# awikner/SPEEDY-ML-1

Hardware: AMD Instinct MI355X
Metric: hybrid timesteps/sec, T30L8 + 1152x6k-node reservoirs; 1/2/4/8-GPU scaling (higher is better)
Workload: dtype f64

## Files before the change

include/speedy_ml.h:

```cpp
#ifndef SPEEDY_ML_H
#define SPEEDY_ML_H

#include <stddef.h>
#include <stdint.h>

#ifdef __cplusplus
extern "C" {
#endif

#define SML_OK 0
#define SML_ERR_ARG (-1)
#define SML_ERR_HIP (-2)
#define SML_ERR_NOMEM (-3)
#define SML_ERR_STATE (-4)
#define SML_ERR_IO (-5)
#define SML_ERR_FORMAT (-6)

#define SML_F32 1
#define SML_F64 2

#define SML_MX 31
#define SML_NX 32
#define SML_MX2 62
#define SML_IX 96
// ... 59 lines not shown
#define SML_RES_PATH_PER_REGION 2
#define SML_RES_PATH_UNGROUPED_FINISH 4
#define SML_RES_PATH_STEPWISE_DRIVE 8
#define SML_RES_PATH_RADIUS_GLOBAL 16
int sml_res_set_reference_paths(sml_reservoirs *c, int flags);
#define SML_RADIUS_OK 0
#define SML_RADIUS_MAXITER 1
#define SML_RADIUS_ZERO 2
#define SML_RADIUS_INVALID 3
int sml_res_spectral_radius(sml_reservoirs *c, double tol, int max_iter, double *lo, double *hi, int *iters,
                            int *info, void *stream);
int sml_gen_region(int n, int k, int ninp, uint64_t seed, int region, double sigma, int *rows, int *cols,
                   float *vals, int *win_col, float *win_val);
int sml_res_set_update_cus(sml_reservoirs *c, int cus);
int sml_res_update_balanced(sml_reservoirs *c, int *balanced);
int sml_res_ell_layout(sml_reservoirs *c, int i, int *a_width, int *a_overflow, int *win_q, int *win_ell);
int sml_res_set_begin_mode(sml_reservoirs *c, int mode);
int sml_res_begin_fused(const sml_reservoirs *c, int *fused);
int sml_res_synchronize(sml_reservoirs *c, const double *d_inputs, int length, int64_t stride, void *stream);
int sml_res_start_prediction(sml_reservoirs *c, const double *d_inputs, int length, int64_t stride,
                             double *d_feedback, void *stream);
int sml_res_train_drive(sml_reservoirs *c, const double *d_inputs, int m, int64_t stride, const double *d_model,
                        int64_t model_stride, double *d_states, double *d_targets, void *stream);
int sml_res_step_host(sml_reservoirs *c, const double *feedback, const double *local_model, double *outvec);
int sml_res_footprint(const sml_reservoirs *c, int64_t *weight_bytes, int64_t *algorithmic_bytes_per_step);
int sml_res_enable_timing(sml_reservoirs *c, int capacity);
int sml_res_kernel_times(sml_reservoirs *c, float *update_ms, float *readout_ms, int max_steps, int *count);
#define SML_RES_MAX_MEMBERS 32
int sml_res_set_members(sml_reservoirs *c, int members);
int sml_res_members(const sml_reservoirs *c, int *members);
// ... 222 lines not shown
```

speedy-ml-1_amd/csrc/sml_res_rows.hpp:

```cpp
#pragma once
#include <hip/hip_runtime.h>

#include <cstdint>

#include "sml_reservoir_layout.hpp"

#ifndef SML_UPD_NT
#define SML_UPD_NT 1
#endif

namespace {
using namespace sml;

__device__ inline int xcd_remap(int b, int nb) {
    const int q8 = nb / 8, rem = nb % 8, xcd = b % 8, idx = b / 8;
    return xcd * q8 + min(xcd, rem) + idx;
}

struct Ell {
    const uint16_t *a_col;
    const void *a_val;
    const uint16_t *w_col;
    const void *w_val;
    const uint64_t *a_om;
// ... 65 lines not shown
        const int np = (rg.a_w + 1) >> 1, n = rg.n;
#pragma unroll
        for (int p = 0; p < kEllA / 2; ++p)
            if (p < np) load_pair<WT, kNT>(q, p, cb + (size_t)p * n + i, vb + 2 * ((size_t)p * n + i));
        if (rg.a_ov) {
            q.om = row_load<kNT>(ell.a_om + rg.a_om + (i >> 6));
            q.ob = row_load<kNT>(ell.a_ob + rg.a_om + (i >> 6));
        }
    }
    if (live && rg.w_w > 0) {
        q.wc = rg.w_q > 0 ? win_col_implicit(rg, i) : (uint32_t)row_load<kNT>(ell.w_col + rg.w_ell + i);
        q.wv = row_load<kNT>((const WT *)ell.w_val + rg.w_ell + i);
    }
}

template <typename WT, int NP, bool OVF>
__device__ inline void load_row_fixed(RowRegs<WT> &q, const RegionDev &rg, const Ell &ell, int i) {
    const uint32_t *cb = reinterpret_cast<const uint32_t *>(ell.a_col + rg.a_ell);
    const WT *vb = (const WT *)ell.a_val + rg.a_ell;
    const uint32_t *zc = reinterpret_cast<const uint32_t *>(ell.zero);
    const WT *zv = reinterpret_cast<const WT *>(ell.zero);
    const int np = (rg.a_w + 1) >> 1, n = rg.n;
    if (OVF) {
        q.om = 0;
        q.ob = 0;
        if (rg.a_ov) {
            q.om = stream_load(ell.a_om + rg.a_om + (i >> 6));
            q.ob = stream_load(ell.a_ob + rg.a_om + (i >> 6));
        }
    }
#pragma unroll
    for (int p = 0; p < NP; ++p) {
        const bool in = p < np;
        load_pair(q, p, in ? cb + (size_t)p * n + i : zc, in ? vb + 2 * ((size_t)p * n + i) : zv);
    }
    if (rg.w_q > 0)
        q.wc = win_col_implicit(rg, i);
    else
        q.wc = stream_load(ell.w_col + rg.w_ell + i);
    q.wv = stream_load((const WT *)ell.w_val + rg.w_ell + i);
}

template <typename WT, bool kFixed>
__device__ inline void resolve_ovf(RowRegs<WT> &q, const RegionDev &rg, const Ell &ell, int i) {
    const int b = i & 63;
    const uint64_t below = b ? q.om << (64 - b) : 0ull;
    q.oh = rg.a_ov && ((q.om >> b) & 1ull);
    const int64_t e = rg.a_oe + q.ob + __popcll(below);
    if (q.oh) {
        q.oc = kFixed ? stream_load(ell.a_oc + e) : ell.a_oc[e];
        q.ov = kFixed ? stream_load((const WT *)ell.a_ov + e) : ((const WT *)ell.a_ov)[e];
    }
}

__device__ __attribute__((always_inline)) inline double res_tanh(double x) {
    double a = fabs(x);
    a = a > 20.0 ? 20.0 : a;
    const double em = expm1(2.0 * a);
    return copysign(em / (em + 2.0), x);
}

template <typename WT>
__device__ inline int ell_col(const RowRegs<WT> &q, int s) {
    return (int)((q.c[s >> 1] >> (16 * (s & 1))) & 0xffffu);
}

template <typename WT>
__device__ __attribute__((always_inline)) inline double ell_row_value(const RowRegs<WT> &q, const RegionDev &rg,
                                                                      const double *xs, const double *fs, int i,
                                                                      double leak) {
    double y = 0.0;
#pragma unroll
    for (int s = 0; s < kEllA; ++s)
        if (s < rg.a_w) y = y + (double)q.v[s] * xs[ell_col(q, s)];
    if (q.oh) y = y + (double)q.ov * xs[q.oc];
    double t = 0.0;
    t = t + (double)q.wv * fs[q.wc];
    const double xn = res_tanh(y + t);
    return (1.0 - leak) * xs[i] + leak * xn;
}

template <typename WT>
struct CsrRows {
    const int32_t *rp;
    const uint16_t *ac;
    const WT *av;
    const int32_t *wp;
    const uint16_t *wc;
    const WT *wv;
};

template <typename WT>
__device__ __attribute__((always_inline)) inline double row_value(RowRegs<WT> &cur, const RegionDev &rg,
                                                                  const Ell &ell, const CsrRows<WT> &csr,
                                                                  const double *xs, const double *fs, int i,
                                                                  double leak) {
    double y = 0.0;
    if (rg.a_w > 0) {
        cur.oh = false;
        if (rg.a_ov) resolve_ovf<WT, false>(cur, rg, ell, i);
#pragma unroll
        for (int s = 0; s < kEllA; ++s)
            if (s < rg.a_w) y = y + (double)cur.v[s] * xs[ell_col(cur, s)];
        if (cur.oh) y = y + (double)cur.ov * xs[cur.oc];
    } else {
        for (int e = csr.rp[i], e1 = csr.rp[i + 1]; e < e1; ++e) y = y + (double)csr.av[e] * xs[csr.ac[e]];
    }
    double t = 0.0;
    if (rg.w_w > 0) {
        t = t + (double)cur.wv * fs[cur.wc];
    } else {
        for (int e = csr.wp[i], e1 = csr.wp[i + 1]; e < e1; ++e) t = t + (double)csr.wv[e] * fs[csr.wc[e]];
    }
    const double xn = res_tanh(y + t);
    return (1.0 - leak) * xs[i] + leak * xn;
// ... 43 lines not shown
```

speedy-ml-1_amd/csrc/sml_res_update.hpp:

```cpp
#pragma once
#include <hip/hip_runtime.h>

#include <cstdint>

#include "sml_res_rows.hpp"
#include "sml_reservoir_layout.hpp"
#include "sml_timeline.hpp"

namespace {
using namespace sml;

template <typename WT, bool kLds, int kMinW = 4>
__global__ __launch_bounds__(kUpdThreads, kMinW) void k_res_update(
    const RegionDev *__restrict__ R, const int32_t *__restrict__ a_rp, const uint16_t *__restrict__ a_col,
    const WT *__restrict__ a_val, const int32_t *__restrict__ w_rp, const uint16_t *__restrict__ w_col,
    const WT *__restrict__ w_val, Ell ell, const double *__restrict__ x_old, double *__restrict__ x_new,
    const double *__restrict__ feedback, double leak, int parts, int lds_x, int nlog) {
    SML_TL_SCOPE(sml::tl::kUpdate);
    extern __shared__ __attribute__((aligned(16))) double smem[];
    const int off = xcd_remap(blockIdx.x, gridDim.x);
    for (int base = 0; base < nlog; base += gridDim.x) {
        const int lb = base + off;
        if (lb < nlog)
            update_block<WT, kLds>(lb, smem, R, a_rp, a_col, a_val, w_rp, w_col, w_val, ell, x_old, x_new,
                                   feedback, leak, parts, lds_x);
        if (base + (int)gridDim.x < nlog) __syncthreads();
    }
}

struct PassDesc {
    int r, base, end, seg;
    bool live;
};

struct StageRegs {
    double x[kStageX];
    double f;
};

template <typename WT, int NP, bool OVF, int kDepth = 2>
__global__ __launch_bounds__(kUpdThreads, 4) void k_res_update_bal(
    const RegionDev *__restrict__ R, const int32_t *__restrict__ row0, const int32_t *__restrict__ blk_r0, int nlocal,
    int64_t total, Ell ell, const double *__restrict__ x_old, double *__restrict__ x_new,
    const double *__restrict__ feedback, double leak, int lds_x, int lds_buf) {
    SML_TL_SCOPE(sml::tl::kUpdate);
    extern __shared__ __attribute__((aligned(16))) double smem[];
    const int G = gridDim.x;
    const int b = xcd_remap(blockIdx.x, G);
    const int g0 = (int)(total * b / G), g1 = (int)(total * (b + 1) / G);
    if (g0 >= g1) return;
    const int tid = threadIdx.x;
    auto seg_at = [&](int r, int seg) -> PassDesc {
        const int a = row0[r], e = row0[r + 1];
        return PassDesc{r, max(g0, a) - a, min(g1, e) - a, seg, true};
    };
    auto succ = [&](const PassDesc &p) -> PassDesc {
        if (!p.live) return p;
        if (p.base + kUpdThreads < p.end) return PassDesc{p.r, p.base + kUpdThreads, p.end, p.seg, true};
        const int r = p.r + 1;
        if (r >= nlocal || row0[r] >= g1) return PassDesc{r, 0, 0, p.seg + 1, false};
        return seg_at(r, p.seg + 1);
    };
    auto load = [&](RowRegs<WT> &q, const PassDesc &p) {
        if (!p.live) return;
        const RegionDev rg = R[p.r];
        const int i = p.base + tid;
        load_row_fixed<WT, NP, OVF>(q, rg, ell, i < p.end ? i : 0);
    };
    auto resolve = [&](RowRegs<WT> &q, const PassDesc &p) {
        q.oh = false;
        if (!OVF || !p.live) return;
        const RegionDev rg = R[p.r];
        if (!rg.a_ov) return;
        const int i = p.base + tid;
        resolve_ovf<WT, true>(q, rg, ell, i < p.end ? i : 0);
    };
    auto stage_load = [&](StageRegs &sr, int r) {
        const RegionDev rg = R[r];
        const double *xo = x_old + rg.x;
#pragma unroll
        for (int q = 0; q < kStageX; ++q) {
            const int j = tid + q * kUpdThreads;
            if (j < rg.n) sr.x[q] = xo[j];
        }
        if (tid < rg.ninp) sr.f = feedback[rg.fb + tid];
    };
    auto stage_store = [&](const StageRegs &sr, int r, double *buf) {
        const RegionDev rg = R[r];
#pragma unroll
        for (int q = 0; q < kStageX; ++q) {
            const int j = tid + q * kUpdThreads;
            if (j < rg.n) buf[j] = sr.x[q];
        }
        if (tid < rg.ninp) buf[lds_x + tid] = sr.f;
    };
    static_assert(kDepth == 2 || kDepth == 3, "update pipeline depth");
    PassDesc P0 = seg_at(blk_r0[b], 0);
    RowRegs<WT> L0, L1, L2, L3;
    load(L0, P0);
    resolve(L0, P0);
    PassDesc P1 = succ(P0);
    load(L1, P1);
    PassDesc P2 = succ(P1), P3 = P2;
    if constexpr (kDepth == 3) {
        load(L2, P2);
        P3 = succ(P2);
    }
    {
        StageRegs sr;
        stage_load(sr, P0.r);
        stage_store(sr, P0.r, smem);
    }
    __syncthreads();
    while (P0.live) {
        resolve(L1, P1);
        if constexpr (kDepth == 3)
            load(L3, P3);
        else
            load(L2, P2);
        const bool newseg = P1.live && P1.seg != P0.seg;
        StageRegs sr;
        if (newseg) stage_load(sr, P1.r);
        {
            const RegionDev rg = R[P0.r];
            const double *xs = smem + (size_t)(P0.seg & 1) * lds_buf, *fs = xs + lds_x;
            const int i = P0.base + tid;
            if (i < P0.end) x_new[rg.x + i] = ell_row_value(L0, rg, xs, fs, i, leak);
        }
        if (newseg) {
            stage_store(sr, P1.r, smem + (size_t)(P1.seg & 1) * lds_buf);
            __syncthreads();
        }
        P0 = P1;
        L0 = L1;
        P1 = P2;
        L1 = L2;
        if constexpr (kDepth == 3) {
            P2 = P3;
            L2 = L3;
            P3 = succ(P3);
        } else {
            P2 = succ(P2);
        }
    }
}

}
```

speedy-ml-1_amd/csrc/sml_reservoir.hip:

```cpp
#include <hip/hip_ext.h>
#include <hip/hip_runtime.h>

#include <algorithm>
#include <cmath>
#include <cstdlib>
#include <cstring>
#include <memory>
#include <new>
#include <type_traits>
#include <vector>

#include "sml_devmem.hpp"
#include "sml_internal.hpp"
#include "sml_reservoir_layout.hpp"
#include "sml_timeline.hpp"

SML_TL_DEFINE(reservoir)

#include "sml_res_rows.hpp"
#include "sml_res_update.hpp"
#include "sml_res_drive.hpp"
#include "sml_res_radius.hpp"
#include "sml_res_tiling.hpp"
#include "sml_res_readout.hpp"
// ... 51 lines not shown
    bool stepwise_drive = false;
    bool radius_global = false;
    double *d_rad_xy = nullptr, *d_rad_part = nullptr;
    RadiusOut *d_rad_out = nullptr;
    StepShape shape;
    int members = 1;
    MemberShape mshape;
    MemberFinish mfin;
    int fin_tile_want = 0;
    int32_t *d_tgt_idx = nullptr;
    const uint64_t *fin_wflag = nullptr;
    uint64_t fin_wval = 0;
    unsigned *fin_wlate = nullptr;
    long long fin_wtimeout = 400000000ll;
    int upd_cus = 0, ncu = 0;
    std::vector<int32_t> blk_off;
    std::vector<std::vector<int32_t>> blk_host;
    int blk_cap = 0;
    size_t max_lds = 0;
    int32_t *d_row0 = nullptr, *d_blk_r0 = nullptr;
    std::vector<int32_t> row0_h;
    int8_t *d_outl = nullptr;
    int32_t *d_asm_dst = nullptr;
    int32_t *d_fb_src = nullptr;
    uint8_t *d_fb_l = nullptr;
    uint16_t *d_fb_reg = nullptr;
    int tot_tisr = 0;
    int32_t *d_tisr_fb = nullptr, *d_tisr_grid = nullptr;
    uint16_t *d_tisr_reg = nullptr;
    int32_t *d_lm_src = nullptr;
    uint8_t *d_lm_l = nullptr;
    double *d_io = nullptr;
    size_t d_io_n = 0;
    StepEvents timers;
    std::vector<double> meanstd_h;
// ... 261 lines not shown
        for (int l = 0; l < kMeanStd; ++l) c->meanstd_h[(size_t)i * 2 * kMeanStd + kMeanStd + l] = 1.0;
    int rc;
    if ((rc = upload(c->d_rd, c->rd)) || (rc = upload(c->d_meanstd, c->meanstd_h)) || (rc = build_tables(c)) ||
        (rc = upload(c->d_row0, c->row0_h)))
        return rc;
    *out = owner.release();
    return SML_OK;
}

Ell make_ell(const sml_reservoirs *c) {
    return Ell{c->d_a_ell_col, c->d_a_ell_val, c->d_w_ell_col, c->d_w_ell_val, c->d_a_om,
               c->d_a_ob,      c->d_a_oc,      c->d_a_ov,      c->d_zero};
}


int launch_update_bal(sml_reservoirs *c, const double *xo, double *xn, const double *d_feedback, hipStream_t st) {
    const StepShape &s = c->shape;
    const int64_t total = c->row0_h[c->nlocal];
    int G = c->upd_cus > 0 ? c->upd_cus : std::max(c->ncu, 1);
    G = (int)std::max<int64_t>(1, std::min<int64_t>(G, total));
    if (G > c->blk_cap) {
        const int cap = std::max(G, std::max(c->ncu, c->upd_cus));
        if (c->d_blk_r0) {
            SML_HIP(hipDeviceSynchronize());
            c->mem.release(&c->d_blk_r0);
            c->blk_cap = 0;
        }
        if (int rc = pool(c, &c->d_blk_r0, (int64_t)cap * (cap + 1) / 2)) return rc;
        c->blk_off.assign(cap + 1, -1);
        c->blk_cap = cap;
    }
    if (c->blk_off[G] < 0) {
        c->blk_off[G] = G * (G - 1) / 2;
        c->blk_host.push_back(block_first_regions(c->row0_h, G));
        SML_HIP(hipMemcpyAsync(c->d_blk_r0 + c->blk_off[G], c->blk_host.back().data(), (size_t)G * 4,
                               hipMemcpyHostToDevice, st));
    }
    const int32_t *blk_r0 = c->d_blk_r0 + c->blk_off[G];
    const Ell ell = make_ell(c);
    int np = 2;
    bool ovf = false;
    for (int i = 0; i < c->nlocal; ++i) {
        np = std::max(np, (c->rd[i].a_w + 1) / 2);
        ovf = ovf || c->rd[i].a_ov;
    }
    auto go = [&](auto kern) {
        hipLaunchKernelGGL(kern, dim3(G), dim3(kUpdThreads), s.lds_bal, st, c->d_rd, c->d_row0, blk_r0, c->nlocal,
                           total, ell, xo, xn, d_feedback, c->leakage, s.lds_x, s.lds_buf);
    };
    with_wt(c, [&](auto tag) {
        using WT = decltype(tag);
        if (np == 2) ovf ? go(k_res_update_bal<WT, 2, true, 2>) : go(k_res_update_bal<WT, 2, false, 2>);
        else if (np == 3) ovf ? go(k_res_update_bal<WT, 3, true, 2>) : go(k_res_update_bal<WT, 3, false, 2>);
        else ovf ? go(k_res_update_bal<WT, 4, true, 2>) : go(k_res_update_bal<WT, 4, false, 2>);
    });
    SML_HIP(hipGetLastError());
    return SML_OK;
}

int launch_update(sml_reservoirs *c, const double *xo, double *xn, const double *d_feedback, hipStream_t st) {
    const StepShape &s = c->shape;
    if (s.balanced) return launch_update_bal(c, xo, xn, d_feedback, st);
    const int nlog = s.parts * c->nlocal;
    const Ell ell = make_ell(c);
    with_wt(c, [&](auto tag) {
        using WT = decltype(tag);
        auto go = [&](auto kern, size_t shared) {
            hipLaunchKernelGGL(kern, dim3(nlog), dim3(kUpdThreads), shared, st, c->d_rd, c->d_a_rp, c->d_a_col,
                               (const WT *)c->d_a_val, c->d_w_rp, c->d_w_col, (const WT *)c->d_w_val, ell, xo, xn,
// ... 348 lines not shown
    return SML_OK;
}

extern "C" int sml_res_set_update_cus(sml_reservoirs *c, int cus) {
    SML_REQUIRE(c && cus >= 0, "bad argument");
    c->upd_cus = cus;
    return SML_OK;
}

extern "C" int sml_res_update_balanced(sml_reservoirs *c, int *balanced) {
    SML_REQUIRE(c && balanced, "null argument");
    *balanced = c->shape.balanced ? 1 : 0;
    return SML_OK;
}

extern "C" int sml_res_ell_layout(sml_reservoirs *c, int i, int *a_width, int *a_overflow, int *win_q,
                                  int *win_ell) {
    if (int rc = check_region(c, i)) return rc;
    SML_REQUIRE(a_width && a_overflow && win_q && win_ell, "null argument");
    const RegionDev &r = c->rd[i];
    *a_width = r.a_w;
    *a_overflow = r.a_ov;
    *win_q = r.w_q;
    *win_ell = r.w_w;
    return SML_OK;
}

extern "C" int sml_res_set_reference_paths(sml_reservoirs *c, int flags) {
    SML_REQUIRE(c && (flags & ~31) == 0, "bad argument");
    const bool csr = flags & SML_RES_PATH_CSR;
// ... 679 lines not shown
```

speedy-ml-1_amd/csrc/sml_reservoir_layout.cpp:

```cpp
#include "sml_reservoir_layout.hpp"

#include <algorithm>

namespace sml {

PoolPlan plan_pools(const PoolPlanIn &in) {
    PoolPlan p;
    p.rd.resize(in.nlocal);
    p.ld.resize(in.nlocal);
    for (int i = 0; i < in.nlocal; ++i) {
        const int n = in.n[i];
        p.ld[i] = (in.ncs + n + kLdAlign - 1) / kLdAlign * kLdAlign;
        RegionDev &r = p.rd[i];
        r.n = n;
        r.ninp = in.ninp[i];
        r.ld = p.ld[i];
        r.a_rp = p.tot_a_rp;
        p.tot_a_rp += n + 1;
        r.a_nz = p.tot_a_nz;
        p.tot_a_nz += in.k[i];
        r.w_rp = p.tot_w_rp;
        p.tot_w_rp += n + 1;
        r.w_nz = p.tot_w_nz;
        p.tot_w_nz += n;
// ... 317 lines not shown
        std::copy(t.begin(), t.begin() + cnt, tidx.begin() + (size_t)i * nout);
    }
    return SML_OK;
}

std::vector<int32_t> block_first_regions(const std::vector<int32_t> &row0, int G) {
    const int64_t total = row0.back();
    std::vector<int32_t> r0(G);
    for (int b = 0; b < G; ++b) {
        const int64_t g0 = total * b / G;
        r0[b] = (int32_t)(std::upper_bound(row0.begin(), row0.end(), (int32_t)g0) - row0.begin() - 1);
    }
    return r0;
}

void footprint(int nlocal, const int *nn, const int *kk, const int *ni, int ncs, int nout, int64_t wb,
               int64_t *weight_bytes, int64_t *algo_bytes) {
    int64_t w = 0, a = 0;
    for (int i = 0; i < nlocal; ++i) {
        const int64_t n = nn[i], k = kk[i], ninp = ni[i];
        const int64_t wout = wb * nout * (ncs + n);
        const int64_t amat = 4 * (n + 1) + (2 + wb) * k;
        const int64_t winm = 4 * (n + 1) + (2 + wb) * n;
        w += wout + amat + winm;
        a += wout + amat + winm + 8 * n + 8 * n + 8 * ninp + 8 * ncs + 8 * nout;
    }
    if (weight_bytes) *weight_bytes = w;
    if (algo_bytes) *algo_bytes = a;
}

// ... 2 lines not shown
```

speedy-ml-1_amd/csrc/sml_reservoir_layout.hpp:

```cpp
#pragma once

#include <cstdint>
#include <vector>

#include "sml_internal.hpp"

namespace sml {

constexpr int kLdAlign = 32;
constexpr int kRows = 8;
constexpr int kMeanStd = 36;
constexpr int kTisrStride = 16;
constexpr int kSrcKeep = -1;

constexpr int kEllA = 8;
constexpr int kEllW = 1;

struct RegionDev {
    int n, ninp, ld;
    int a_w, w_w;
    int a_ov;
    int w_q;
    uint32_t w_magic;
    int64_t a_rp, a_nz, w_rp, w_nz, wout, x, xaug, fb;
// ... 149 lines not shown
    std::vector<uint16_t> fb_reg;
    std::vector<int32_t> lm_src;
    std::vector<uint8_t> lm_l;
    std::vector<int32_t> tisr_fb, tisr_grid;
    std::vector<uint16_t> tisr_reg;
    std::vector<int8_t> outl;
    std::vector<int32_t> tgt_idx;
};

int build_region_tables(const TablesIn &in, RegionTables *out);

int out_std_index(int o, const RegionGeom &g);

std::vector<int32_t> block_first_regions(const std::vector<int32_t> &row0, int G);

void footprint(int nlocal, const int *n, const int *k, const int *ninp, int ncs, int nout, int64_t wb,
               int64_t *weight_bytes, int64_t *algo_bytes);

}
```

speedy-ml-1_amd/speedy_ml_amd/_lib.py:

```python
from __future__ import annotations

import ctypes
import os
import subprocess

PKG_ROOT = os.path.dirname(os.path.dirname(os.path.abspath(__file__)))
LIB_PATH = os.environ.get("SML_LIB") or os.path.join(PKG_ROOT, "lib", "libspeedyml.so")
CSRC = os.path.join(PKG_ROOT, "csrc")

SML_OK = 0
SML_F32 = 1
SML_F64 = 2

EXPORTED = (
    "sml_last_error", "sml_abi_version",
    "sml_spectral_create", "sml_spectral_destroy", "sml_spectral_tables",
    "sml_grid_batched", "sml_spec_batched", "sml_gridy_batched", "sml_gridx_batched",
    "sml_specx_batched", "sml_specy_batched", "sml_vdspec_batched", "sml_uvspec_batched",
    "sml_grid_host", "sml_spec_host",
    "sml_res_create", "sml_res_destroy", "sml_res_ninp", "sml_res_feedback_offsets",
    "sml_res_load_region_f32", "sml_res_load_region_f64", "sml_res_set_state", "sml_res_get_state",
    "sml_res_step", "sml_res_step_begin", "sml_res_step_finish", "sml_res_step_finish_grid", "sml_res_step_finish_assemble", "sml_res_step_host", "sml_res_synchronize",
    "sml_res_footprint", "sml_res_enable_timing", "sml_res_kernel_times", "sml_res_set_read_waves",
    "sml_res_set_begin_mode", "sml_res_begin_fused",
# ... 12 lines not shown
    "sml_dyn_run_model", "sml_dyn_last_safe", "sml_dyn_set_check_cus", "sml_res_info",
    "sml_comm_unique_id", "sml_comm_create", "sml_comm_create_file", "sml_comm_destroy", "sml_comm_rank",
    "sml_comm_allgather",
    "sml_hybrid_create", "sml_hybrid_destroy", "sml_hybrid_set_buffers", "sml_hybrid_set_tisr",
    "sml_hybrid_streams", "sml_hybrid_cus", "sml_hybrid_start", "sml_hybrid_predict", "sml_hybrid_advance", "sml_hybrid_step",
    "sml_hybrid_run_speedy", "sml_hybrid_sync",
    "sml_device_alloc", "sml_device_free", "sml_copy_to_device", "sml_copy_to_host", "sml_region_geometry",
    "sml_processor_decomposition", "sml_hybrid_set_tisr_table", "sml_tisr_date_index", "sml_res_tile_tisr_field",
    "sml_res_create_generic", "sml_res_step_slab", "sml_res_start_prediction",
    "sml_comm_create_local", "sml_exchange_plan", "sml_hybrid_advance_slabs", "sml_hybrid_set_hop_mode",
    "sml_hybrid_hop_mode", "sml_calendar_delta_hour", "sml_hybrid_set_feb29", "sml_hybrid_get_feb29",
    "sml_res_mean_std", "sml_res_set_outvec_ld", "sml_hybrid_set_slab", "sml_hybrid_start_slab",
    "sml_hybrid_exchange_width", "sml_hybrid_slab_buffers", "sml_dyn_set_hybrid_sst", "sml_dyn_set_sea_ice",
    "sml_hybrid_set_pipelined", "sml_res_step_cancel", "sml_res_step_begun", "sml_hybrid_set_force_exchange",
    "sml_hybrid_exchanges", "sml_hybrid_set_chain", "sml_hybrid_chain", "sml_hybrid_exchange_stream",
    "sml_res_set_update_cus", "sml_res_update_balanced", "sml_probe_mfma_f64_clock", "sml_res_ell_layout",
    "sml_dyn_get_sea_ice", "sml_dyn_get_physics", "sml_dyn_get_forcing", "sml_dyn_set_surface",
    "sml_dyn_set_climatology", "sml_dyn_fordate", "sml_dyn_fordate_ex", "sml_dyn_fordate_count",
    "sml_hybrid_set_calendar", "sml_hybrid_window_date", "sml_hybrid_set_hop_timeout",
    "sml_dyn_set_check_timeout", "sml_dyn_check_stream", "sml_dyn_set_fused", "sml_res_set_reference_paths",
    "sml_train_set_panel", "sml_res_train_drive", "sml_region_target_index",
    "sml_res_spectral_radius", "sml_gen_region",
    "sml_res_set_members", "sml_res_members", "sml_res_set_state_member", "sml_res_get_state_member",
    "sml_res_step_members", "sml_res_synchronize_members", "sml_res_member_tile",
    "sml_res_step_begin_members", "sml_res_step_finish_members", "sml_res_step_finish_grid_members",
    "sml_res_step_finish_assemble_members", "sml_res_member_finish_tile",
    "sml_res_tile_feedback_members", "sml_res_tile_tisr_field_members",
    "sml_slab_create", "sml_slab_destroy", "sml_slab_info", "sml_slab_start", "sml_slab_predict", "sml_slab_sst",
    "sml_slab_ring", "sml_slab_buffers",
    "sml_ens_create", "sml_ens_destroy", "sml_ens_info", "sml_ens_reset", "sml_ens_moments", "sml_ens_scores",
    "sml_ens_read", "sml_ens_weights",
# ... 176 lines not shown
        "sml_hybrid_set_slab": [vp, vp, vp, vp, i, i, d],
        "sml_hybrid_start_slab": [vp, vp],
        "sml_hybrid_exchange_width": [vp, ip],
        "sml_hybrid_slab_buffers": [vp, pp, pp, ip, pp, pp],
        "sml_dyn_set_hybrid_sst": [vp, vp, d, vp],
        "sml_dyn_set_sea_ice": [vp, vp, vp],
        "sml_res_step_cancel": [vp],
        "sml_res_step_begun": [vp, ip],
        "sml_hybrid_set_force_exchange": [vp, i],
        "sml_hybrid_exchanges": [vp, i64p],
        "sml_hybrid_set_chain": [vp, i],
        "sml_hybrid_chain": [vp, ip, ip],
        "sml_hybrid_exchange_stream": [vp, pp],
        "sml_res_set_update_cus": [vp, i],
        "sml_res_update_balanced": [vp, ip],
        "sml_res_ell_layout": [vp, i, ip, ip, ip, ip],
        "sml_probe_mfma_f64_clock": [i, ctypes.POINTER(ctypes.c_double), ctypes.POINTER(ctypes.c_double)],
        "sml_dyn_get_sea_ice": [vp, vp, vp],
        "sml_dyn_get_physics": [vp, vp],
        "sml_dyn_get_forcing": [vp, vp, vp, vp],
        "sml_dyn_set_surface": [vp, vp],
        "sml_dyn_set_climatology": [vp, vp],
        "sml_dyn_fordate": [vp, i, i, i, vp],
        "sml_dyn_fordate_ex": [vp, i, i, i, i, vp],
        "sml_dyn_fordate_count": [vp, ip],
        "sml_hybrid_set_calendar": [vp, i, ctypes.c_int64, i],
        "sml_hybrid_window_date": [vp, ip],
        "sml_hybrid_set_hop_timeout": [vp, ctypes.c_int64],
        "sml_res_train_drive": [vp, vp, i, ctypes.c_int64, vp, ctypes.c_int64, vp, vp, vp],
        "sml_region_target_index": [i, i, i, vp, ip],
# ... 57 lines not shown
```

speedy-ml-1_amd/speedy_ml_amd/reservoir.py:

```python
from __future__ import annotations

import ctypes
import os

import numpy as np

from ._lib import SML_F32, SML_F64, check, lib, ptr, stream_ptr
from .domain import CHUNK_PRED, CHUNK_SPEEDY, NUM_REGIONS


class Reservoirs:

    def __init__(self, region_ids, sst_flags, n, k, numregions: int = NUM_REGIONS,
                 chunk_speedy: int = CHUNK_SPEEDY, nout: int = CHUNK_PRED, weight_dtype: str = "f32",
                 leakage: float = 1.0, ninp=None, out_index=None):
        self.region_ids = np.ascontiguousarray(region_ids, dtype=np.int32)
        self.sst = np.ascontiguousarray(sst_flags, dtype=np.uint8)
        self.n = np.ascontiguousarray(n, dtype=np.int32)
        self.k = np.ascontiguousarray(k, dtype=np.int32)
        self.nlocal = len(self.region_ids)
        self.numregions = numregions
        self.ncs = chunk_speedy
        self.nout = nout
        self.weight_dtype = weight_dtype
# ... 235 lines not shown
    def set_read_waves(self, waves: int):
        check(lib().sml_res_set_read_waves(self._h, int(waves)))

    def set_outvec_ld(self, ld: int):
        check(lib().sml_res_set_outvec_ld(self._h, int(ld)))
        self._ov_ld = int(ld)

    def set_update_cus(self, cus: int):
        check(lib().sml_res_set_update_cus(self._h, int(cus)))

    def update_balanced(self) -> bool:
        b = ctypes.c_int()
        check(lib().sml_res_update_balanced(self._h, ctypes.byref(b)))
        return bool(b.value)

    def ell_layout(self, i: int) -> dict:
        v = [ctypes.c_int() for _ in range(4)]
        check(lib().sml_res_ell_layout(self._h, int(i), *[ctypes.byref(x) for x in v]))
        return dict(a_width=v[0].value, a_overflow=bool(v[1].value), win_q=v[2].value, win_ell=bool(v[3].value))

    def set_reference_paths(self, csr: bool = False, per_region: bool = False, ungrouped_finish: bool = False,
                            stepwise_drive: bool = False, radius_global: bool = False):
        flags = ((1 if csr else 0) | (2 if per_region else 0) | (4 if ungrouped_finish else 0)
                 | (8 if stepwise_drive else 0) | (16 if radius_global else 0))
        check(lib().sml_res_set_reference_paths(self._h, flags))

    def spectral_radius(self, tol: float = 2e-14, max_iter: int = 1000, stream=None):
        lo, hi = np.zeros(self.nlocal), np.zeros(self.nlocal)
        iters, info = np.zeros(self.nlocal, dtype=np.int32), np.zeros(self.nlocal, dtype=np.int32)
        check(lib().sml_res_spectral_radius(self._h, float(tol), int(max_iter), ptr(lo), ptr(hi), ptr(iters),
# ... 129 lines not shown
```

Before: 1236.

## Drive balanced reservoir update from precomputed pass table with branchless pipelined loads

The balanced update kernel no longer computes segment boundaries on the fly. It reads a host-built per-block table of passes that carries new-segment and buffer-parity flags, padded so the loop can unroll three stages with a rotating register set and prefetch overflow words further ahead. Loads become branch-free: masked offsets point at a zero buffer, and input-column recomputation is specialised away when every region uses implicit columns. The aim is to cut scalar control overhead and keep more memory loads in flight, at the cost of a device table per grid size, more kernel variants and higher register pressure.

```diff
diff --git a/include/speedy_ml.h b/include/speedy_ml.h
--- a/include/speedy_ml.h
+++ b/include/speedy_ml.h
@@ -97,6 +97,7 @@
                    float *vals, int *win_col, float *win_val);
 int sml_res_set_update_cus(sml_reservoirs *c, int cus);
 int sml_res_update_balanced(sml_reservoirs *c, int *balanced);
+int sml_res_update_form(sml_reservoirs *c, int *pairs, int *overflow, int *win_implicit);
 int sml_res_ell_layout(sml_reservoirs *c, int i, int *a_width, int *a_overflow, int *win_q, int *win_ell);
 int sml_res_set_begin_mode(sml_reservoirs *c, int mode);
 int sml_res_begin_fused(const sml_reservoirs *c, int *fused);
diff --git a/speedy-ml-1_amd/csrc/sml_res_rows.hpp b/speedy-ml-1_amd/csrc/sml_res_rows.hpp
--- a/speedy-ml-1_amd/csrc/sml_res_rows.hpp
+++ b/speedy-ml-1_amd/csrc/sml_res_rows.hpp
@@ -103,42 +103,83 @@
     }
 }
 
-template <typename WT, int NP, bool OVF>
-__device__ inline void load_row_fixed(RowRegs<WT> &q, const RegionDev &rg, const Ell &ell, int i) {
+
+struct OvfWord {
+    uint64_t om;
+    uint32_t ob;
+};
+
+template <typename WT, int NP>
+struct BalRegs {
+    uint32_t c[NP];
+    WT v[2 * NP];
+    uint32_t wc;
+    WT wv;
+    OvfWord w;
+    uint32_t oc;
+    WT ov;
+    bool oh;
+};
+
+template <typename T>
+__device__ inline T stream_at(const T *base, uint32_t byte_off) {
+    return stream_load(reinterpret_cast<const T *>(reinterpret_cast<const char *>(base) + byte_off));
+}
+
+__device__ inline void load_ovf_word(OvfWord &w, const RegionDev &rg, const Ell &ell, int i) {
+    const bool has = rg.a_ov != 0;
+    const uint32_t m = has ? ~0u : 0u, wi = (uint32_t)i >> 6;
+    w.om = stream_at(has ? ell.a_om + rg.a_om : reinterpret_cast<const uint64_t *>(ell.zero), (wi << 3) & m);
+    w.ob = stream_at(has ? ell.a_ob + rg.a_om : reinterpret_cast<const uint32_t *>(ell.zero), (wi << 2) & m);
+}
+
+template <typename WT, int NP, bool kImpl>
+__device__ inline void load_row_fixed(BalRegs<WT, NP> &q, const RegionDev &rg, const Ell &ell, int i) {
+    typedef typename Pair<WT>::N V2;
     const uint32_t *cb = reinterpret_cast<const uint32_t *>(ell.a_col + rg.a_ell);
     const WT *vb = (const WT *)ell.a_val + rg.a_ell;
-    const uint32_t *zc = reinterpret_cast<const uint32_t *>(ell.zero);
-    const WT *zv = reinterpret_cast<const WT *>(ell.zero);
     const int np = (rg.a_w + 1) >> 1, n = rg.n;
-    if (OVF) {
-        q.om = 0;
-        q.ob = 0;
-        if (rg.a_ov) {
-            q.om = stream_load(ell.a_om + rg.a_om + (i >> 6));
-            q.ob = stream_load(ell.a_ob + rg.a_om + (i >> 6));
-        }
-    }
+    const uint32_t oc = (uint32_t)i * 4u, ov = (uint32_t)i * (uint32_t)sizeof(V2), ow = (uint32_t)i * (uint32_t)sizeof(WT);
 #pragma unroll
     for (int p = 0; p < NP; ++p) {
-        const bool in = p < np;
-        load_pair(q, p, in ? cb + (size_t)p * n + i : zc, in ? vb + 2 * ((size_t)p * n + i) : zv);
-    }
-    if (rg.w_q > 0)
-        q.wc = win_col_implicit(rg, i);
-    else
-        q.wc = stream_load(ell.w_col + rg.w_ell + i);
-    q.wv = stream_load((const WT *)ell.w_val + rg.w_ell + i);
-}
-
-template <typename WT, bool kFixed>
+        const bool in = p == 0 || p < np;
+        const uint32_t m = in ? ~0u : 0u;
+        q.c[p] = stream_at(in ? cb + (size_t)p * n : reinterpret_cast<const uint32_t *>(ell.zero), oc & m);
+        const V2 v = stream_at(in ? reinterpret_cast<const V2 *>(vb + 2 * (size_t)p * n)
+                                  : reinterpret_cast<const V2 *>(ell.zero), ov & m);
+        q.v[2 * p] = v.x;
+        q.v[2 * p + 1] = v.y;
+    }
+    if constexpr (!kImpl) {
+        const bool stored = rg.w_q <= 0;
+        q.wc = stream_at(stored ? ell.w_col + rg.w_ell : reinterpret_cast<const uint16_t *>(ell.zero),
+                         ((uint32_t)i * 2u) & (stored ? ~0u : 0u));
+    }
+    q.wv = stream_at((const WT *)ell.w_val + rg.w_ell, ow);
+}
+
+template <typename WT, int NP>
+__device__ inline void resolve_ovf_fixed(BalRegs<WT, NP> &q, const OvfWord &w, const RegionDev &rg, const Ell &ell,
+                                         int i) {
+    const bool has = rg.a_ov != 0;
+    const int b = i & 63;
+    const uint64_t below = b ? w.om << (64 - b) : 0ull;
+    q.oh = has && ((w.om >> b) & 1ull);
+    const uint32_t e = q.oh ? w.ob + (uint32_t)__popcll(below) : 0u;
+    q.oc = stream_at(has ? ell.a_oc + rg.a_oe : reinterpret_cast<const uint16_t *>(ell.zero), e * 2u);
+    q.ov = stream_at(has ? (const WT *)ell.a_ov + rg.a_oe : reinterpret_cast<const WT *>(ell.zero),
+                     e * (uint32_t)sizeof(WT));
+}
+
+template <typename WT>
 __device__ inline void resolve_ovf(RowRegs<WT> &q, const RegionDev &rg, const Ell &ell, int i) {
     const int b = i & 63;
     const uint64_t below = b ? q.om << (64 - b) : 0ull;
     q.oh = rg.a_ov && ((q.om >> b) & 1ull);
     const int64_t e = rg.a_oe + q.ob + __popcll(below);
     if (q.oh) {
-        q.oc = kFixed ? stream_load(ell.a_oc + e) : ell.a_oc[e];
-        q.ov = kFixed ? stream_load((const WT *)ell.a_ov + e) : ((const WT *)ell.a_ov)[e];
+        q.oc = ell.a_oc[e];
+        q.ov = ((const WT *)ell.a_ov)[e];
     }
 }
 
@@ -149,24 +190,47 @@
     return copysign(em / (em + 2.0), x);
 }
 
-template <typename WT>
-__device__ inline int ell_col(const RowRegs<WT> &q, int s) {
+template <typename Q>
+__device__ inline int ell_col(const Q &q, int s) {
     return (int)((q.c[s >> 1] >> (16 * (s & 1))) & 0xffffu);
 }
 
-template <typename WT>
-__device__ __attribute__((always_inline)) inline double ell_row_value(const RowRegs<WT> &q, const RegionDev &rg,
+template <typename WT, int NP, bool OVF, bool kImpl>
+__device__ __attribute__((always_inline)) inline double ell_row_value(const BalRegs<WT, NP> &q, const RegionDev &rg,
                                                                       const double *xs, const double *fs, int i,
                                                                       double leak) {
+    uint32_t wc = win_col_implicit(rg, i);
+    if constexpr (!kImpl) wc = rg.w_q > 0 ? wc : q.wc;
+    constexpr bool kTight = sizeof(WT) == 8 && NP == 4;
+    constexpr int kG = kTight ? 1 : 2 * NP;
+    double xv[kG], xo = 0.0, fv = 0.0, xi = 0.0;
+    if constexpr (!kTight) {
+        if constexpr (OVF) xo = xs[q.oc];
+        fv = fs[wc];
+        xi = xs[i];
+    }
     double y = 0.0;
 #pragma unroll
-    for (int s = 0; s < kEllA; ++s)
-        if (s < rg.a_w) y = y + (double)q.v[s] * xs[ell_col(q, s)];
-    if (q.oh) y = y + (double)q.ov * xs[q.oc];
+    for (int s0 = 0; s0 < 2 * NP; s0 += kG) {
+#pragma unroll
+        for (int s = 0; s < kG; ++s) xv[s] = xs[ell_col(q, s0 + s)];
+#pragma unroll
+        for (int s = 0; s < kG; ++s) {
+            const double ys = y + (double)q.v[s0 + s] * xv[s];
+            y = s0 + s < rg.a_w ? ys : y;
+        }
+    }
+    if constexpr (OVF) {
+        if constexpr (kTight) xo = xs[q.oc];
+        const double ys = y + (double)q.ov * xo;
+        y = q.oh ? ys : y;
+    }
+    if constexpr (kTight) fv = fs[wc];
     double t = 0.0;
-    t = t + (double)q.wv * fs[q.wc];
+    t = t + (double)q.wv * fv;
     const double xn = res_tanh(y + t);
-    return (1.0 - leak) * xs[i] + leak * xn;
+    if constexpr (kTight) xi = xs[i];
+    return (1.0 - leak) * xi + leak * xn;
 }
 
 template <typename WT>
@@ -187,7 +251,7 @@
     double y = 0.0;
     if (rg.a_w > 0) {
         cur.oh = false;
-        if (rg.a_ov) resolve_ovf<WT, false>(cur, rg, ell, i);
+        if (rg.a_ov) resolve_ovf(cur, rg, ell, i);
 #pragma unroll
         for (int s = 0; s < kEllA; ++s)
             if (s < rg.a_w) y = y + (double)cur.v[s] * xs[ell_col(cur, s)];
diff --git a/speedy-ml-1_amd/csrc/sml_res_update.hpp b/speedy-ml-1_amd/csrc/sml_res_update.hpp
--- a/speedy-ml-1_amd/csrc/sml_res_update.hpp
+++ b/speedy-ml-1_amd/csrc/sml_res_update.hpp
@@ -28,52 +28,43 @@
     }
 }
 
-struct PassDesc {
-    int r, base, end, seg;
-    bool live;
-};
-
 struct StageRegs {
     double x[kStageX];
     double f;
 };
 
-template <typename WT, int NP, bool OVF, int kDepth = 2>
+template <typename WT, int NP, bool OVF, bool kImpl>
 __global__ __launch_bounds__(kUpdThreads, 4) void k_res_update_bal(
-    const RegionDev *__restrict__ R, const int32_t *__restrict__ row0, const int32_t *__restrict__ blk_r0, int nlocal,
-    int64_t total, Ell ell, const double *__restrict__ x_old, double *__restrict__ x_new,
-    const double *__restrict__ feedback, double leak, int lds_x, int lds_buf) {
+    const RegionDev *__restrict__ R, const int32_t *__restrict__ tab, int hdr, Ell ell,
+    const double *__restrict__ x_old, double *__restrict__ x_new, const double *__restrict__ feedback, double leak,
+    int lds_x, int lds_buf) {
     SML_TL_SCOPE(sml::tl::kUpdate);
     extern __shared__ __attribute__((aligned(16))) double smem[];
-    const int G = gridDim.x;
-    const int b = xcd_remap(blockIdx.x, G);
-    const int g0 = (int)(total * b / G), g1 = (int)(total * (b + 1) / G);
-    if (g0 >= g1) return;
+    static_assert(kUpdUnroll == 3 && kUpdAhead == 4, "the stages below read entries j .. j + 4, three to a trip");
+    const int b = xcd_remap(blockIdx.x, gridDim.x);
+    const int t0 = tab[b], npass = tab[b + 1] - t0 - kUpdAhead;
+    if (npass <= 0) return;
+    const UpdatePass *T = reinterpret_cast<const UpdatePass *>(tab + hdr) + t0;
     const int tid = threadIdx.x;
-    auto seg_at = [&](int r, int seg) -> PassDesc {
-        const int a = row0[r], e = row0[r + 1];
-        return PassDesc{r, max(g0, a) - a, min(g1, e) - a, seg, true};
+    typedef BalRegs<WT, NP> Regs;
+    constexpr int kWordAhead = sizeof(WT) == 4 ? 2 : 1;
+    auto row = [&](const UpdatePass &p) {
+        const int i = p.base + tid;
+        return i < p.end ? i : 0;
     };
-    auto succ = [&](const PassDesc &p) -> PassDesc {
-        if (!p.live) return p;
-        if (p.base + kUpdThreads < p.end) return PassDesc{p.r, p.base + kUpdThreads, p.end, p.seg, true};
-        const int r = p.r + 1;
-        if (r >= nlocal || row0[r] >= g1) return PassDesc{r, 0, 0, p.seg + 1, false};
-        return seg_at(r, p.seg + 1);
+    auto load_word = [&](OvfWord &w, const UpdatePass &p) {
+        if constexpr (OVF) load_ovf_word(w, R[p.r], ell, row(p));
     };
-    auto load = [&](RowRegs<WT> &q, const PassDesc &p) {
-        if (!p.live) return;
+    auto load = [&](Regs &q, const UpdatePass &p) {
         const RegionDev rg = R[p.r];
-        const int i = p.base + tid;
-        load_row_fixed<WT, NP, OVF>(q, rg, ell, i < p.end ? i : 0);
+        load_row_fixed<WT, NP, kImpl>(q, rg, ell, row(p));
     };
-    auto resolve = [&](RowRegs<WT> &q, const PassDesc &p) {
+    auto resolve = [&](Regs &q, const OvfWord &w, const UpdatePass &p) {
         q.oh = false;
-        if (!OVF || !p.live) return;
-        const RegionDev rg = R[p.r];
-        if (!rg.a_ov) return;
-        const int i = p.base + tid;
-        resolve_ovf<WT, true>(q, rg, ell, i < p.end ? i : 0);
+        if constexpr (OVF) {
+            const RegionDev rg = R[p.r];
+            resolve_ovf_fixed(q, w, rg, ell, row(p));
+        }
     };
     auto stage_load = [&](StageRegs &sr, int r) {
         const RegionDev rg = R[r];
@@ -81,9 +72,9 @@
 #pragma unroll
         for (int q = 0; q < kStageX; ++q) {
             const int j = tid + q * kUpdThreads;
-            if (j < rg.n) sr.x[q] = xo[j];
+            sr.x[q] = xo[j < rg.n ? j : 0];
         }
-        if (tid < rg.ninp) sr.f = feedback[rg.fb + tid];
+        sr.f = feedback[rg.fb + (tid < rg.ninp ? tid : 0)];
     };
     auto stage_store = [&](const StageRegs &sr, int r, double *buf) {
         const RegionDev rg = R[r];
@@ -94,54 +85,48 @@
         }
         if (tid < rg.ninp) buf[lds_x + tid] = sr.f;
     };
-    static_assert(kDepth == 2 || kDepth == 3, "update pipeline depth");
-    PassDesc P0 = seg_at(blk_r0[b], 0);
-    RowRegs<WT> L0, L1, L2, L3;
-    load(L0, P0);
-    resolve(L0, P0);
-    PassDesc P1 = succ(P0);
-    load(L1, P1);
-    PassDesc P2 = succ(P1), P3 = P2;
-    if constexpr (kDepth == 3) {
-        load(L2, P2);
-        P3 = succ(P2);
-    }
-    {
+    auto buffer = [&](const UpdatePass &p) { return smem + (p.flags & kPassOdd ? (size_t)lds_buf : 0); };
+    auto compute = [&](const Regs &q, const UpdatePass &p) {
+        const RegionDev rg = R[p.r];
+        const double *xs = buffer(p), *fs = xs + lds_x;
+        const int i = p.base + tid;
+        if (i < p.end) x_new[rg.x + i] = ell_row_value<WT, NP, OVF, kImpl>(q, rg, xs, fs, i, leak);
+    };
+    auto stage = [&](Regs &cur, Regs &mid, Regs &far, int j) {
+        const UpdatePass p0 = T[j], p1 = T[j + 1], p2 = T[j + 2], pw = T[j + 2 + kWordAhead];
+        const bool newseg = p1.flags & kPassNewSeg;
         StageRegs sr;
-        stage_load(sr, P0.r);
-        stage_store(sr, P0.r, smem);
-    }
-    __syncthreads();
-    while (P0.live) {
-        resolve(L1, P1);
-        if constexpr (kDepth == 3)
-            load(L3, P3);
-        else
-            load(L2, P2);
-        const bool newseg = P1.live && P1.seg != P0.seg;
-        StageRegs sr;
-        if (newseg) stage_load(sr, P1.r);
-        {
-            const RegionDev rg = R[P0.r];
-            const double *xs = smem + (size_t)(P0.seg & 1) * lds_buf, *fs = xs + lds_x;
-            const int i = P0.base + tid;
-            if (i < P0.end) x_new[rg.x + i] = ell_row_value(L0, rg, xs, fs, i, leak);
-        }
+        if (newseg) stage_load(sr, p1.r);
+        resolve(far, far.w, p2);
+        load_word(kWordAhead == 2 ? mid.w : cur.w, pw);
+        load(far, p2);
+        compute(cur, p0);
         if (newseg) {
-            stage_store(sr, P1.r, smem + (size_t)(P1.seg & 1) * lds_buf);
+            stage_store(sr, p1.r, buffer(p1));
             __syncthreads();
         }
-        P0 = P1;
-        L0 = L1;
-        P1 = P2;
-        L1 = L2;
-        if constexpr (kDepth == 3) {
-            P2 = P3;
-            L2 = L3;
-            P3 = succ(P3);
-        } else {
-            P2 = succ(P2);
-        }
+    };
+    Regs A, B, C;
+    {
+        const UpdatePass p0 = T[0], p1 = T[1], p2 = T[2], p3 = T[3];
+        load_word(A.w, p0);
+        load(A, p0);
+        resolve(A, A.w, p0);
+        load_word(B.w, p1);
+        load(B, p1);
+        resolve(B, B.w, p1);
+        load_word(C.w, p2);
+        if constexpr (kWordAhead == 2) load_word(A.w, p3);
+        StageRegs sr;
+        stage_load(sr, p0.r);
+        stage_store(sr, p0.r, smem);
+        __builtin_amdgcn_s_waitcnt(0x0F70);
+        __syncthreads();
+    }
+    for (int j = 0; j < npass; j += kUpdUnroll) {
+        stage(A, B, C, j);
+        stage(B, C, A, j + 1);
+        stage(C, A, B, j + 2);
     }
 }
 
diff --git a/speedy-ml-1_amd/csrc/sml_reservoir.hip b/speedy-ml-1_amd/csrc/sml_reservoir.hip
--- a/speedy-ml-1_amd/csrc/sml_reservoir.hip
+++ b/speedy-ml-1_amd/csrc/sml_reservoir.hip
@@ -89,11 +89,10 @@
     unsigned *fin_wlate = nullptr;
     long long fin_wtimeout = 400000000ll;
     int upd_cus = 0, ncu = 0;
-    std::vector<int32_t> blk_off;
-    std::vector<std::vector<int32_t>> blk_host;
-    int blk_cap = 0;
+    std::vector<int32_t *> d_pass;
+    std::vector<std::vector<int32_t>> pass_host;
     size_t max_lds = 0;
-    int32_t *d_row0 = nullptr, *d_blk_r0 = nullptr;
+    int32_t *d_row0 = nullptr;
     std::vector<int32_t> row0_h;
     int8_t *d_outl = nullptr;
     int32_t *d_asm_dst = nullptr;
@@ -385,45 +384,52 @@
 }
 
 
+struct UpdateForm {
+    int np;
+    bool ovf, implicit;
+};
+
+UpdateForm update_form(const sml_reservoirs *c) {
+    UpdateForm f{2, false, true};
+    for (int i = 0; i < c->nlocal; ++i) {
+        f.np = std::max(f.np, (c->rd[i].a_w + 1) / 2);
+        f.ovf = f.ovf || c->rd[i].a_ov;
+        f.implicit = f.implicit && c->rd[i].w_q > 0;
+    }
+    return f;
+}
+
 int launch_update_bal(sml_reservoirs *c, const double *xo, double *xn, const double *d_feedback, hipStream_t st) {
     const StepShape &s = c->shape;
     const int64_t total = c->row0_h[c->nlocal];
     int G = c->upd_cus > 0 ? c->upd_cus : std::max(c->ncu, 1);
     G = (int)std::max<int64_t>(1, std::min<int64_t>(G, total));
-    if (G > c->blk_cap) {
-        const int cap = std::max(G, std::max(c->ncu, c->upd_cus));
-        if (c->d_blk_r0) {
-            SML_HIP(hipDeviceSynchronize());
-            c->mem.release(&c->d_blk_r0);
-            c->blk_cap = 0;
-        }
-        if (int rc = pool(c, &c->d_blk_r0, (int64_t)cap * (cap + 1) / 2)) return rc;
-        c->blk_off.assign(cap + 1, -1);
-        c->blk_cap = cap;
-    }
-    if (c->blk_off[G] < 0) {
-        c->blk_off[G] = G * (G - 1) / 2;
-        c->blk_host.push_back(block_first_regions(c->row0_h, G));
-        SML_HIP(hipMemcpyAsync(c->d_blk_r0 + c->blk_off[G], c->blk_host.back().data(), (size_t)G * 4,
-                               hipMemcpyHostToDevice, st));
-    }
-    const int32_t *blk_r0 = c->d_blk_r0 + c->blk_off[G];
+    if ((int)c->d_pass.size() <= G) c->d_pass.resize(G + 1, nullptr);
+    if (!c->d_pass[G]) {
+        c->pass_host.push_back(update_pass_table(c->row0_h, G));
+        const std::vector<int32_t> &t = c->pass_host.back();
+        if (int rc = pool(c, &c->d_pass[G], (int64_t)t.size())) return rc;
+        SML_HIP(hipMemcpyAsync(c->d_pass[G], t.data(), t.size() * 4, hipMemcpyHostToDevice, st));
+    }
     const Ell ell = make_ell(c);
-    int np = 2;
-    bool ovf = false;
-    for (int i = 0; i < c->nlocal; ++i) {
-        np = std::max(np, (c->rd[i].a_w + 1) / 2);
-        ovf = ovf || c->rd[i].a_ov;
-    }
+    const UpdateForm f = update_form(c);
     auto go = [&](auto kern) {
-        hipLaunchKernelGGL(kern, dim3(G), dim3(kUpdThreads), s.lds_bal, st, c->d_rd, c->d_row0, blk_r0, c->nlocal,
-                           total, ell, xo, xn, d_feedback, c->leakage, s.lds_x, s.lds_buf);
+        hipLaunchKernelGGL(kern, dim3(G), dim3(kUpdThreads), s.lds_bal, st, c->d_rd, c->d_pass[G],
+                           update_pass_header(G), ell, xo, xn, d_feedback, c->leakage, s.lds_x, s.lds_buf);
     };
     with_wt(c, [&](auto tag) {
         using WT = decltype(tag);
-        if (np == 2) ovf ? go(k_res_update_bal<WT, 2, true, 2>) : go(k_res_update_bal<WT, 2, false, 2>);
-        else if (np == 3) ovf ? go(k_res_update_bal<WT, 3, true, 2>) : go(k_res_update_bal<WT, 3, false, 2>);
-        else ovf ? go(k_res_update_bal<WT, 4, true, 2>) : go(k_res_update_bal<WT, 4, false, 2>);
+        auto pick = [&](auto np, auto ovf) {
+            constexpr int kNp = decltype(np)::value;
+            constexpr bool kOvf = decltype(ovf)::value;
+            f.implicit ? go(k_res_update_bal<WT, kNp, kOvf, true>) : go(k_res_update_bal<WT, kNp, kOvf, false>);
+        };
+        auto width = [&](auto np) {
+            f.ovf ? pick(np, std::true_type{}) : pick(np, std::false_type{});
+        };
+        if (f.np == 2) width(std::integral_constant<int, 2>{});
+        else if (f.np == 3) width(std::integral_constant<int, 3>{});
+        else width(std::integral_constant<int, 4>{});
     });
     SML_HIP(hipGetLastError());
     return SML_OK;
@@ -802,6 +808,15 @@
     return SML_OK;
 }
 
+extern "C" int sml_res_update_form(sml_reservoirs *c, int *pairs, int *overflow, int *win_implicit) {
+    SML_REQUIRE(c && pairs && overflow && win_implicit, "null argument");
+    const UpdateForm f = update_form(c);
+    *pairs = f.np;
+    *overflow = f.ovf ? 1 : 0;
+    *win_implicit = f.implicit ? 1 : 0;
+    return SML_OK;
+}
+
 extern "C" int sml_res_ell_layout(sml_reservoirs *c, int i, int *a_width, int *a_overflow, int *win_q,
                                   int *win_ell) {
     if (int rc = check_region(c, i)) return rc;
diff --git a/speedy-ml-1_amd/csrc/sml_reservoir_layout.cpp b/speedy-ml-1_amd/csrc/sml_reservoir_layout.cpp
--- a/speedy-ml-1_amd/csrc/sml_reservoir_layout.cpp
+++ b/speedy-ml-1_amd/csrc/sml_reservoir_layout.cpp
@@ -355,6 +355,37 @@
     return r0;
 }
 
+std::vector<int32_t> update_pass_table(const std::vector<int32_t> &row0, int G) {
+    const int64_t total = row0.back();
+    const int nlocal = (int)row0.size() - 1, hdr = update_pass_header(G);
+    std::vector<int32_t> t((size_t)hdr, 0);
+    auto push = [&t](int32_t r, int32_t base, int32_t end, int32_t flags) {
+        const int32_t e[4] = {r, base, end, flags};
+        t.insert(t.end(), e, e + 4);
+    };
+    int r = 0;
+    for (int b = 0; b < G; ++b) {
+        t[b] = (int32_t)((t.size() - hdr) / 4);
+        const int64_t g0 = total * b / G, g1 = total * (b + 1) / G;
+        if (g0 >= g1) continue;
+        while (row0[r + 1] <= g0) ++r;
+        int live = 0, seg = 0, last_r = r;
+        for (int q = r; q < nlocal && row0[q] < g1; ++q) {
+            const int32_t a = row0[q], e = row0[q + 1];
+            if (a == e) continue;
+            const int32_t base = (int32_t)(std::max<int64_t>(g0, a) - a), end = (int32_t)(std::min<int64_t>(g1, e) - a);
+            for (int32_t p = base; p < end; p += kUpdThreads, ++live)
+                push(q, p, end, (seg & 1 ? kPassOdd : 0) | (p == base && seg > 0 ? kPassNewSeg : 0));
+            last_r = q;
+            ++seg;
+        }
+        const int pad = (kUpdUnroll - live % kUpdUnroll) % kUpdUnroll + kUpdAhead;
+        for (int p = 0; p < pad; ++p) push(last_r, 0, 0, (seg - 1) & 1 ? kPassOdd : 0);
+    }
+    t[G] = (int32_t)((t.size() - hdr) / 4);
+    return t;
+}
+
 void footprint(int nlocal, const int *nn, const int *kk, const int *ni, int ncs, int nout, int64_t wb,
                int64_t *weight_bytes, int64_t *algo_bytes) {
     int64_t w = 0, a = 0;
diff --git a/speedy-ml-1_amd/csrc/sml_reservoir_layout.hpp b/speedy-ml-1_amd/csrc/sml_reservoir_layout.hpp
--- a/speedy-ml-1_amd/csrc/sml_reservoir_layout.hpp
+++ b/speedy-ml-1_amd/csrc/sml_reservoir_layout.hpp
@@ -187,6 +187,18 @@
 
 std::vector<int32_t> block_first_regions(const std::vector<int32_t> &row0, int G);
 
+constexpr int kUpdUnroll = 3;
+constexpr int kUpdAhead = 4;
+struct UpdatePass {
+    int32_t r;
+    int32_t base, end;
+    int32_t flags;
+};
+constexpr int32_t kPassNewSeg = 1;
+constexpr int32_t kPassOdd = 2;
+inline int update_pass_header(int G) { return (G + 1 + 3) / 4 * 4; }
+std::vector<int32_t> update_pass_table(const std::vector<int32_t> &row0, int G);
+
 void footprint(int nlocal, const int *n, const int *k, const int *ninp, int ncs, int nout, int64_t wb,
                int64_t *weight_bytes, int64_t *algo_bytes);
 
diff --git a/speedy-ml-1_amd/speedy_ml_amd/_lib.py b/speedy-ml-1_amd/speedy_ml_amd/_lib.py
--- a/speedy-ml-1_amd/speedy_ml_amd/_lib.py
+++ b/speedy-ml-1_amd/speedy_ml_amd/_lib.py
@@ -50,7 +50,7 @@
     "sml_hybrid_exchange_width", "sml_hybrid_slab_buffers", "sml_dyn_set_hybrid_sst", "sml_dyn_set_sea_ice",
     "sml_hybrid_set_pipelined", "sml_res_step_cancel", "sml_res_step_begun", "sml_hybrid_set_force_exchange",
     "sml_hybrid_exchanges", "sml_hybrid_set_chain", "sml_hybrid_chain", "sml_hybrid_exchange_stream",
-    "sml_res_set_update_cus", "sml_res_update_balanced", "sml_probe_mfma_f64_clock", "sml_res_ell_layout",
+    "sml_res_set_update_cus", "sml_res_update_balanced", "sml_res_update_form", "sml_probe_mfma_f64_clock", "sml_res_ell_layout",
     "sml_dyn_get_sea_ice", "sml_dyn_get_physics", "sml_dyn_get_forcing", "sml_dyn_set_surface",
     "sml_dyn_set_climatology", "sml_dyn_fordate", "sml_dyn_fordate_ex", "sml_dyn_fordate_count",
     "sml_hybrid_set_calendar", "sml_hybrid_window_date", "sml_hybrid_set_hop_timeout",
@@ -257,6 +257,7 @@
         "sml_hybrid_exchange_stream": [vp, pp],
         "sml_res_set_update_cus": [vp, i],
         "sml_res_update_balanced": [vp, ip],
+        "sml_res_update_form": [vp, ip, ip, ip],
         "sml_res_ell_layout": [vp, i, ip, ip, ip, ip],
         "sml_probe_mfma_f64_clock": [i, ctypes.POINTER(ctypes.c_double), ctypes.POINTER(ctypes.c_double)],
         "sml_dyn_get_sea_ice": [vp, vp, vp],
diff --git a/speedy-ml-1_amd/speedy_ml_amd/reservoir.py b/speedy-ml-1_amd/speedy_ml_amd/reservoir.py
--- a/speedy-ml-1_amd/speedy_ml_amd/reservoir.py
+++ b/speedy-ml-1_amd/speedy_ml_amd/reservoir.py
@@ -273,6 +273,11 @@
         check(lib().sml_res_update_balanced(self._h, ctypes.byref(b)))
         return bool(b.value)
 
+    def update_form(self) -> dict:
+        p, o, w = ctypes.c_int(), ctypes.c_int(), ctypes.c_int()
+        check(lib().sml_res_update_form(self._h, ctypes.byref(p), ctypes.byref(o), ctypes.byref(w)))
+        return {"pairs": p.value, "overflow": bool(o.value), "win_implicit": bool(w.value)}
+
     def ell_layout(self, i: int) -> dict:
         v = [ctypes.c_int() for _ in range(4)]
         check(lib().sml_res_ell_layout(self._h, int(i), *[ctypes.byref(x) for x in v]))
```

After: 1230. About the same (-0.5%).
